# indrajeetadityaroy9/vit-bias-aware-structural-distillation

Measured on AMD Instinct MI355X. Metric: images/sec BASD train step, DeiT-T student / ViT-B teacher bs=256, higher is better.
Workload: dtype bf16; 1 GPU; BASELINE configs[1]: DeiT-Tiny/16 student, ViT-Base/16 teacher (random init), 224x224, E=4 extraction points, loss linalg fp32/fp64; global_batch=256, per_gpu_batch=256, parallelism=dp1, grad_checkpointing=False

## Files before the change

vit-bias-aware-structural-distillation_amd/csrc/attention.hip:

```cpp
#include "basd_frag.h"

namespace basd {

__device__ __forceinline__ unsigned short f32_to_bf16_rne(float f) {
  unsigned int u = __float_as_uint(f);
  u += 0x7fffu + ((u >> 16) & 1u);
  return (unsigned short)(u >> 16);
}

template <int CTRL> __device__ __forceinline__ float at_dpp_add(float v) {
  return v + __int_as_float(__builtin_amdgcn_update_dpp(0, __float_as_int(v), CTRL, 0xF, 0xF, true));
}

struct RelBias {
  const float* table;
  int gh, gw;
};


template <int NKT, int AT_HD, bool QMEAN = false, bool RELBIAS = false, bool ROPE = false>
__global__ __launch_bounds__(256) __attribute__((amdgpu_waves_per_eu(2, 2))) void attention_fwd_kernel(const unsigned short* __restrict__ qkv, int T, int H,
                                                            float scale, unsigned short* __restrict__ out,
                                                            float* __restrict__ importance, float* __restrict__ lse,
                                                            RelBias rb) {
  static_assert(!(QMEAN && RELBIAS), "the relative-position bias comes with the CLS tap only");
  static_assert(!ROPE || (!QMEAN && !RELBIAS && AT_HD == 64), "the rotary embedding: CLS tap, no bias, whole 32-deep steps");
  constexpr int NKS = (NKT + 1) / 2;
  constexpr int KROWS = 32 * NKS;
  constexpr int NDS = (AT_HD + 31) / 32;
  constexpr int NDT = AT_HD / 16;
  constexpr int NCH = AT_HD / 8;
  constexpr int NCHP = NDS * 4;
  constexpr int AT_LD = NDS * 32 + 8;
  extern __shared__ __align__(16) unsigned short sm[];
  unsigned short* Ks = sm;
  unsigned short* Vs = Ks + KROWS * AT_LD;
  unsigned short* Os = Vs + KROWS * AT_LD;
  int* koff = reinterpret_cast<int*>(Os + 4 * 16 * AT_LD);
  float* tab = reinterpret_cast<float*>(koff + KROWS);
  const int tid = threadIdx.x, lane = tid & 63, wave = tid >> 6;
  const int li = lane & 15, g = lane >> 4;
  const int b = blockIdx.x / H, h = blockIdx.x - b * H;
  const size_t row = (size_t)3 * H * AT_HD;
  const unsigned short* base = qkv + (size_t)b * T * row + (size_t)h * AT_HD;

  constexpr int NLD = (KROWS * NCHP + 255) / 256;
  uint4 kreg[NLD], vreg[NLD];
  float4 kcs[ROPE ? NLD : 1][2];
#pragma unroll
  for (int i = 0; i < NLD; ++i) {
    const int idx = tid + 256 * i;
    const int r = idx / NCHP, c8 = idx - r * NCHP;
    kreg[i] = make_uint4(0, 0, 0, 0);
    vreg[i] = make_uint4(0, 0, 0, 0);
    if constexpr (ROPE) kcs[i][0] = kcs[i][1] = make_float4(0.f, 0.f, 0.f, 0.f);
    if (r < T && c8 < NCH) {
      const unsigned short* p = base + (size_t)r * row + c8 * 8;
      kreg[i] = *reinterpret_cast<const uint4*>(p + (size_t)H * AT_HD);
      vreg[i] = *reinterpret_cast<const uint4*>(p + (size_t)2 * H * AT_HD);
      if constexpr (ROPE) {
        const float4* cs = reinterpret_cast<const float4*>(rb.table + (size_t)r * AT_HD + c8 * 8);
        kcs[i][0] = cs[0];
        kcs[i][1] = cs[1];
      }
    }
  }
  const int R = RELBIAS ? (2 * rb.gh - 1) * (2 * rb.gw - 1) + 3 : 0;
  const int rl = RELBIAS ? 2 * rb.gw - 1 : 0;
  if constexpr (RELBIAS) {
    constexpr int NTAB = (1084 + 255) / 256;
    float tv[NTAB];
#pragma unroll
    for (int i = 0; i < NTAB; ++i) tv[i] = (tid + 256 * i < R) ? rb.table[(size_t)(tid + 256 * i) * H + h] : 0.f;
#pragma unroll
    for (int i = 0; i < NTAB; ++i)
      if (tid + 256 * i < R) tab[tid + 256 * i] = tv[i];
    for (int key = tid; key < KROWS; key += 256) {
      const int yk = (key >= 1 && key < T) ? (key - 1) / rb.gw : 0;
      koff[key] = (key >= 1 && key < T) ? yk * rl + (key - 1 - yk * rb.gw) : 0;
    }
  }
#pragma unroll
  for (int i = 0; i < NLD; ++i) {
    const int idx = tid + 256 * i;
    const int r = idx / NCHP, c8 = idx - r * NCHP;
    if constexpr (ROPE) kreg[i] = rope_chunk(kreg[i], kcs[i][0], kcs[i][1]);
    if (idx < KROWS * NCHP) {
      *reinterpret_cast<uint4*>(Ks + r * AT_LD + c8 * 8) = kreg[i];
      *reinterpret_cast<uint4*>(Vs + r * AT_LD + c8 * 8) = vreg[i];
    }
  }
  __syncthreads();

  const float sl2 = RELBIAS ? 1.4426950408889634f : scale * 1.4426950408889634f;
  const int nqt = (T + 15) >> 4;
  const int full_tiles = T >> 4;
  unsigned short* Ow = Os + wave * 16 * AT_LD;
  auto load_q = [&](int qt_, uint4 (&dst)[NDS], float4 (&cs)[ROPE ? NDS : 1][2]) {
#pragma unroll
    for (int ks = 0; ks < NDS; ++ks) {
      dst[ks] = make_uint4(0, 0, 0, 0);
      if constexpr (ROPE) cs[ks][0] = cs[ks][1] = make_float4(0.f, 0.f, 0.f, 0.f);
      if (qt_ < nqt && qt_ * 16 + li < T && 32 * ks + 8 * g < AT_HD) {
        dst[ks] = *reinterpret_cast<const uint4*>(base + (size_t)(qt_ * 16 + li) * row + 32 * ks + 8 * g);
        if constexpr (ROPE) {
          const float4* p = reinterpret_cast<const float4*>(rb.table + (size_t)(qt_ * 16 + li) * AT_HD + 32 * ks + 8 * g);
          cs[ks][0] = p[0];
          cs[ks][1] = p[1];
        }
      }
    }
  };
  uint4 qnext[NDS];
  float4 qcs[ROPE ? NDS : 1][2];
  load_q(wave, qnext, qcs);
  float csum[QMEAN ? NKT : 1][4];
#pragma unroll
  for (int kt = 0; kt < (QMEAN ? NKT : 1); ++kt)
#pragma unroll
    for (int r = 0; r < 4; ++r) csum[kt][r] = 0.f;
  for (int qt = wave; qt < nqt; qt += 4) {
    const int q0 = qt * 16;
    bf16x8 qf[NDS];
#pragma unroll
    for (int ks = 0; ks < NDS; ++ks) {
      if constexpr (ROPE) qnext[ks] = rope_chunk(qnext[ks], qcs[ks][0], qcs[ks][1]);
      qf[ks] = *reinterpret_cast<bf16x8*>(&qnext[ks]);
    }
    load_q(qt + 4, qnext, qcs);
    f32x4 s[NKT];
#pragma unroll
    for (int kt = 0; kt < NKT; ++kt) {
      f32x4 acc = {0.f, 0.f, 0.f, 0.f};
#pragma unroll
      for (int ks = 0; ks < NDS; ++ks) {
        const uint4 kk = *reinterpret_cast<const uint4*>(Ks + (16 * kt + li) * AT_LD + 32 * ks + 8 * g);
        acc = __builtin_amdgcn_mfma_f32_16x16x32_bf16(*reinterpret_cast<const bf16x8*>(&kk), qf[ks], acc, 0, 0, 0);
      }
      s[kt] = acc;
      if ((kt & 3) == 3) __builtin_amdgcn_sched_barrier(0);
    }
    if constexpr (RELBIAS) {
      const int qi = q0 + li;
      const bool qcls = qi == 0 || qi >= T;
      const int yq = qcls ? 0 : (qi - 1) / rb.gw;
      const int qb = qcls ? R - 3 : (yq + rb.gh - 1) * rl + (qi - 1 - yq * rb.gw) + rb.gw - 1;
      const int c0 = qcls ? R - 1 : R - 2;
#pragma unroll
      for (int kt = 0; kt < NKT; ++kt) {
        const int4 ko = *reinterpret_cast<const int4*>(koff + 16 * kt + 4 * g);
        const int kk[4] = {ko.x, ko.y, ko.z, ko.w};
#pragma unroll
        for (int r = 0; r < 4; ++r) {
          int idx = qcls ? qb : qb - kk[r];
          if (kt == 0 && r == 0 && g == 0) idx = c0;
          s[kt][r] = fmaf(s[kt][r], scale, tab[idx]);
        }
      }
    }
    if (!QMEAN && !RELBIAS && !ROPE && importance != nullptr && qt == 0) {
      float lr[NKT][4];
      float tmx = -3.0e38f;
#pragma unroll
      for (int kt = 0; kt < NKT; ++kt)
#pragma unroll
        for (int r = 0; r < 4; r += 2) {
          const unsigned int w = pack_bf16(s[kt][r], s[kt][r + 1]);
          lr[kt][r] = __uint_as_float(w << 16) * scale;
          lr[kt][r + 1] = __uint_as_float(w & 0xffff0000u) * scale;
          if (kt >= full_tiles) {
            if (16 * kt + 4 * g + r >= T) lr[kt][r] = -3.0e38f;
            if (16 * kt + 4 * g + r + 1 >= T) lr[kt][r + 1] = -3.0e38f;
          }
          tmx = fmaxf(tmx, fmaxf(lr[kt][r], lr[kt][r + 1]));
        }
      tmx = fmaxf(tmx, __shfl_xor(tmx, 16, 64));
      tmx = fmaxf(tmx, __shfl_xor(tmx, 32, 64));
      float tsum = 0.f;
#pragma unroll
      for (int kt = 0; kt < NKT; ++kt)
#pragma unroll
        for (int r = 0; r < 4; ++r) {
          lr[kt][r] = __builtin_amdgcn_exp2f((lr[kt][r] - tmx) * 1.4426950408889634f);
          tsum += lr[kt][r];
        }
      tsum += __shfl_xor(tsum, 16, 64);
      tsum += __shfl_xor(tsum, 32, 64);
      if (li == 0) {
        const float tinv = 1.f / (tsum * (float)H);
#pragma unroll
        for (int kt = 0; kt < NKT; ++kt)
#pragma unroll
          for (int r = 0; r < 4; ++r) {
            const int key = 16 * kt + 4 * g + r;
            if (key >= 1 && (kt < full_tiles || key < T))
              importance[((size_t)b * H + h) * (T - 1) + key - 1] = lr[kt][r] * tinv;
          }
      }
    }
    float mx = -3.0e38f;
#pragma unroll
    for (int kt = 0; kt < NKT; ++kt)
#pragma unroll
      for (int r = 0; r < 4; ++r) {
        if (kt >= full_tiles && 16 * kt + 4 * g + r >= T) s[kt][r] = -3.0e38f;
        mx = fmaxf(mx, s[kt][r]);
      }
    mx = fmaxf(mx, __shfl_xor(mx, 16, 64));
    mx = fmaxf(mx, __shfl_xor(mx, 32, 64));
    float sum = 0.f;
#pragma unroll
    for (int kt = 0; kt < NKT; ++kt)
#pragma unroll
      for (int r = 0; r < 4; ++r) {
        const float p = __builtin_amdgcn_exp2f((s[kt][r] - mx) * sl2);
        s[kt][r] = p;
        sum += p;
      }
    sum += __shfl_xor(sum, 16, 64);
    sum += __shfl_xor(sum, 32, 64);
    const float inv = 1.f / sum;
    if constexpr (RELBIAS || ROPE) {
      if (importance != nullptr && qt == 0 && li == 0) {
        const float tinv = inv / (float)H;
#pragma unroll
        for (int kt = 0; kt < NKT; ++kt)
#pragma unroll
          for (int r = 0; r < 4; ++r) {
            const int key = 16 * kt + 4 * g + r;
            if (key >= 1 && key < T) importance[((size_t)b * H + h) * (T - 1) + key - 1] = s[kt][r] * tinv;
          }
      }
    }
    if constexpr (QMEAN) {
      const float qinv = (q0 + li < T) ? inv : 0.f;
#pragma unroll
      for (int kt = 0; kt < NKT; ++kt)
#pragma unroll
        for (int r = 0; r < 4; ++r) csum[kt][r] = fmaf(s[kt][r], qinv, csum[kt][r]);
    }
    if (!RELBIAS && lse != nullptr && g == 0 && q0 + li < T) lse[((size_t)b * H + h) * T + q0 + li] = fmaf(mx, scale, __logf(sum));
    f32x4 o[NDT];
#pragma unroll
    for (int dt = 0; dt < NDT; ++dt) o[dt] = (f32x4){0.f, 0.f, 0.f, 0.f};
#pragma unroll
    for (int ks = 0; ks < NKS; ++ks) {
      const int K1 = (2 * ks + 1 < NKT) ? 2 * ks + 1 : 0;
      uint4 pw;
      pw.x = pack_bf16(s[2 * ks][0] * inv, s[2 * ks][1] * inv);
      pw.y = pack_bf16(s[2 * ks][2] * inv, s[2 * ks][3] * inv);
      pw.z = (2 * ks + 1 < NKT) ? pack_bf16(s[K1][0] * inv, s[K1][1] * inv) : 0u;
      pw.w = (2 * ks + 1 < NKT) ? pack_bf16(s[K1][2] * inv, s[K1][3] * inv) : 0u;
      const bf16x8 pa = *reinterpret_cast<const bf16x8*>(&pw);
      const int qq = li >> 2, pp = li & 3;
#pragma unroll
      for (int dt = 0; dt < NDT; ++dt) {
        const unsigned short* a0 = Vs + (32 * ks + 4 * g + qq) * AT_LD + 16 * dt + 4 * pp;
        const v4s lo = __builtin_amdgcn_ds_read_tr16_b64_v4i16((lds_v4s*)a0);
        const v4s hi = __builtin_amdgcn_ds_read_tr16_b64_v4i16((lds_v4s*)(a0 + 16 * AT_LD));
        const bf16x8 vb = {lo[0], lo[1], lo[2], lo[3], hi[0], hi[1], hi[2], hi[3]};
        o[dt] = __builtin_amdgcn_mfma_f32_16x16x32_bf16(pa, vb, o[dt], 0, 0, 0);
      }
    }
#pragma unroll
    for (int dt = 0; dt < NDT; ++dt)
#pragma unroll
      for (int r = 0; r < 4; r += 2) {
        const unsigned int w = pack_bf16(o[dt][r], o[dt][r + 1]);
        Ow[(4 * g + r) * AT_LD + 16 * dt + li] = (unsigned short)(w & 0xffffu);
        Ow[(4 * g + r + 1) * AT_LD + 16 * dt + li] = (unsigned short)(w >> 16);
      }
    __builtin_amdgcn_s_waitcnt(0xc07f);
#pragma unroll
    for (int c = 0; c < (16 * NCH + 63) / 64; ++c) {
      const int idx = lane + 64 * c, r = idx / NCH, c8 = idx - r * NCH;
      if (idx < 16 * NCH && q0 + r < T) {
        const uint4 v = *reinterpret_cast<const uint4*>(Ow + r * AT_LD + c8 * 8);
        *reinterpret_cast<uint4*>(out + ((size_t)(b * T + q0 + r) * H + h) * AT_HD + c8 * 8) = v;
      }
    }
    __builtin_amdgcn_s_waitcnt(0xc07f);
  }
  if constexpr (QMEAN) {
    float* cw = reinterpret_cast<float*>(Os) + wave * (16 * AT_LD / 2);
#pragma unroll
    for (int kt = 0; kt < NKT; ++kt)
#pragma unroll
      for (int r = 0; r < 4; ++r) {
        float v = csum[kt][r];
        v = at_dpp_add<0xB1>(v);
        v = at_dpp_add<0x4E>(v);
        v = at_dpp_add<0x124>(v);
        v = at_dpp_add<0x128>(v);
        if (li == 0) cw[16 * kt + 4 * g + r] = v;
      }
    __syncthreads();
    const float* c0 = reinterpret_cast<const float*>(Os);
    const float norm = 1.f / ((float)H * (float)T);
    for (int key = tid; key < T; key += 256) {
      float v = 0.f;
#pragma unroll
      for (int w = 0; w < 4; ++w) v += c0[w * (16 * AT_LD / 2) + key];
      importance[((size_t)b * H + h) * T + key] = v * norm;
    }
  }
}

template <int NKT, int HD, bool QMEAN = false, bool RELBIAS = false, bool ROPE = false>
static void launch_attention(const void* qkv, int B, int T, int H, float scale, void* out, float* importance,
                             float* lse, hipStream_t st, RelBias rb = RelBias{nullptr, 0, 0}) {
  constexpr int KROWS = 32 * ((NKT + 1) / 2);
  constexpr int LD = (HD + 31) / 32 * 32 + 8;
  size_t lds = ((size_t)2 * KROWS * LD + 4 * 16 * LD) * sizeof(unsigned short);
  static_assert(8 * LD >= KROWS, "the output staging tile of a wave holds its query-mean column sums");
  static_assert((2 * KROWS * LD + 4 * 16 * LD) % 8 == 0, "the key offsets behind the tiles are read 16 bytes at a time");
  if (RELBIAS) lds += ((size_t)KROWS + (size_t)(2 * rb.gh - 1) * (2 * rb.gw - 1) + 3) * sizeof(float);
  allow_full_lds((const void*)attention_fwd_kernel<NKT, HD, QMEAN, RELBIAS, ROPE>);
  hipLaunchKernelGGL((attention_fwd_kernel<NKT, HD, QMEAN, RELBIAS, ROPE>), dim3(B * H), dim3(256), lds, st,
                     (const unsigned short*)qkv, T, H, scale, (unsigned short*)out, importance, lse, rb);
}

}

extern "C" int basd_attention_fwd_bf16(const void* qkv, int B, int T, int H, int hd, float scale, void* out,
                                       float* importance, float* lse, void* stream) {
  using namespace basd;
  if (B <= 0) return BASD_OK;
  if ((hd != 64 && hd != 80) || T < 1 || T > 272 || H < 1)
    return fail(BASD_ERR_SHAPE, "attention_fwd: T=%d H=%d hd=%d unsupported (hd 64 | 80, T <= 272)", T, H, hd);
  if (importance != nullptr && T < 2) return fail(BASD_ERR_SHAPE, "attention_fwd: importance needs T >= 2");
  hipStream_t st = (hipStream_t)stream;
  if (hd == 64) {
    if (T <= 64) launch_attention<4, 64>(qkv, B, T, H, scale, out, importance, lse, st);
    else if (T <= 208) launch_attention<13, 64>(qkv, B, T, H, scale, out, importance, lse, st);
    else launch_attention<17, 64>(qkv, B, T, H, scale, out, importance, lse, st);
  } else {
    if (T <= 208) launch_attention<13, 80>(qkv, B, T, H, scale, out, importance, lse, st);
    else launch_attention<17, 80>(qkv, B, T, H, scale, out, importance, lse, st);
  }
  return check_launch("attention_fwd");
}

extern "C" int basd_attention_fwd_qmean_bf16(const void* qkv, int B, int T, int H, int hd, float scale, void* out,
                                             float* importance, void* stream) {
  using namespace basd;
  if (B <= 0) return BASD_OK;
  if ((hd != 64 && hd != 80) || T < 1 || T > 272 || H < 1)
    return fail(BASD_ERR_SHAPE, "attention_fwd_qmean: T=%d H=%d hd=%d unsupported (hd 64 | 80, T <= 272)", T, H, hd);
  if (importance == nullptr) return fail(BASD_ERR_SHAPE, "attention_fwd_qmean: importance is required");
  hipStream_t st = (hipStream_t)stream;
  if (hd == 64) {
    if (T <= 64) launch_attention<4, 64, true>(qkv, B, T, H, scale, out, importance, nullptr, st);
    else if (T <= 208) launch_attention<13, 64, true>(qkv, B, T, H, scale, out, importance, nullptr, st);
    else launch_attention<17, 64, true>(qkv, B, T, H, scale, out, importance, nullptr, st);
  } else {
    if (T <= 208) launch_attention<13, 80, true>(qkv, B, T, H, scale, out, importance, nullptr, st);
    else launch_attention<17, 80, true>(qkv, B, T, H, scale, out, importance, nullptr, st);
  }
  return check_launch("attention_fwd_qmean");
}

extern "C" int basd_attention_fwd_relbias_bf16(const void* qkv, const float* table, int B, int gh, int gw, int H, int hd,
                                               float scale, void* out, float* importance, void* stream) {
  using namespace basd;
  if (hd != 64 || gh < 1 || gw < 1 || gh > 271 || gw > 271 || gh * gw > 271 || H < 1)
    return fail(BASD_ERR_SHAPE, "attention_fwd_relbias: grid %d x %d H=%d hd=%d unsupported (hd 64, 2 <= gh * gw + 1 <= 272)",
                gh, gw, H, hd);
  if (B <= 0) return BASD_OK;
  const int T = gh * gw + 1;
  const RelBias rb{table, gh, gw};
  hipStream_t st = (hipStream_t)stream;
  if (T <= 64) launch_attention<4, 64, false, true>(qkv, B, T, H, scale, out, importance, nullptr, st, rb);
  else if (T <= 208) launch_attention<13, 64, false, true>(qkv, B, T, H, scale, out, importance, nullptr, st, rb);
  else launch_attention<17, 64, false, true>(qkv, B, T, H, scale, out, importance, nullptr, st, rb);
  return check_launch("attention_fwd_relbias");
}

extern "C" int basd_attention_fwd_rope_bf16(const void* qkv, const float* rope, int B, int T, int H, int hd, float scale,
                                            void* out, float* importance, void* stream) {
  using namespace basd;
  if (hd != 64 || T < 2 || T > 272 || H < 1 || B < 1 || rope == nullptr)
    return fail(BASD_ERR_SHAPE, "attention_fwd_rope: B=%d T=%d H=%d hd=%d rope=%s unsupported (hd 64, 2 <= T <= 272, B, H >= 1, "
                                "a table)", B, T, H, hd, rope == nullptr ? "NULL" : "given");
  const RelBias rb{rope, 0, 0};
  hipStream_t st = (hipStream_t)stream;
  if (T <= 64) launch_attention<4, 64, false, false, true>(qkv, B, T, H, scale, out, importance, nullptr, st, rb);
  else if (T <= 208) launch_attention<13, 64, false, false, true>(qkv, B, T, H, scale, out, importance, nullptr, st, rb);
  else launch_attention<17, 64, false, false, true>(qkv, B, T, H, scale, out, importance, nullptr, st, rb);
  return check_launch("attention_fwd_rope");
}
```

Measured before the change: 8161 images/sec.

## Software-pipeline K/V LDS reads, rebalance query tiles, and coalesce importance stores

Result: no change. 8181 images/sec (median of 6 runs) (+0.2%).

```diff
diff --git a/vit-bias-aware-structural-distillation_amd/csrc/attention.hip b/vit-bias-aware-structural-distillation_amd/csrc/attention.hip
--- a/vit-bias-aware-structural-distillation_amd/csrc/attention.hip
+++ b/vit-bias-aware-structural-distillation_amd/csrc/attention.hip
@@ -32,6 +32,10 @@
   constexpr int NCH = AT_HD / 8;
   constexpr int NCHP = NDS * 4;
   constexpr int AT_LD = NDS * 32 + 8;
+  constexpr bool TIGHT = NKT == 17 && AT_HD == 80;
+  constexpr int KD = TIGHT ? (QMEAN ? 1 : 2) : 4;
+  constexpr int VD = TIGHT ? (QMEAN ? 0 : 1) : 2;
+  constexpr int SCHED_PIN = 0x2 | 0x4 | 0x10 | 0x400;
   extern __shared__ __align__(16) unsigned short sm[];
   unsigned short* Ks = sm;
   unsigned short* Vs = Ks + KROWS * AT_LD;
@@ -65,37 +69,10 @@
       }
     }
   }
-  const int R = RELBIAS ? (2 * rb.gh - 1) * (2 * rb.gw - 1) + 3 : 0;
-  const int rl = RELBIAS ? 2 * rb.gw - 1 : 0;
-  if constexpr (RELBIAS) {
-    constexpr int NTAB = (1084 + 255) / 256;
-    float tv[NTAB];
-#pragma unroll
-    for (int i = 0; i < NTAB; ++i) tv[i] = (tid + 256 * i < R) ? rb.table[(size_t)(tid + 256 * i) * H + h] : 0.f;
-#pragma unroll
-    for (int i = 0; i < NTAB; ++i)
-      if (tid + 256 * i < R) tab[tid + 256 * i] = tv[i];
-    for (int key = tid; key < KROWS; key += 256) {
-      const int yk = (key >= 1 && key < T) ? (key - 1) / rb.gw : 0;
-      koff[key] = (key >= 1 && key < T) ? yk * rl + (key - 1 - yk * rb.gw) : 0;
-    }
-  }
-#pragma unroll
-  for (int i = 0; i < NLD; ++i) {
-    const int idx = tid + 256 * i;
-    const int r = idx / NCHP, c8 = idx - r * NCHP;
-    if constexpr (ROPE) kreg[i] = rope_chunk(kreg[i], kcs[i][0], kcs[i][1]);
-    if (idx < KROWS * NCHP) {
-      *reinterpret_cast<uint4*>(Ks + r * AT_LD + c8 * 8) = kreg[i];
-      *reinterpret_cast<uint4*>(Vs + r * AT_LD + c8 * 8) = vreg[i];
-    }
-  }
-  __syncthreads();
-
-  const float sl2 = RELBIAS ? 1.4426950408889634f : scale * 1.4426950408889634f;
   const int nqt = (T + 15) >> 4;
-  const int full_tiles = T >> 4;
-  unsigned short* Ow = Os + wave * 16 * AT_LD;
+  const int nround = nqt >> 2;
+  const int wextra = 4 * nround + ((wave + 3) & 3);
+  auto tile_of = [&](int i) { return (QMEAN || i < nround) ? wave + 4 * i : (i == nround ? wextra : nqt); };
   auto load_q = [&](int qt_, uint4 (&dst)[NDS], float4 (&cs)[ROPE ? NDS : 1][2]) {
 #pragma unroll
     for (int ks = 0; ks < NDS; ++ks) {
@@ -113,13 +90,58 @@
   };
   uint4 qnext[NDS];
   float4 qcs[ROPE ? NDS : 1][2];
-  load_q(wave, qnext, qcs);
+  load_q(tile_of(0), qnext, qcs);
+  const int R = RELBIAS ? (2 * rb.gh - 1) * (2 * rb.gw - 1) + 3 : 0;
+  const int rl = RELBIAS ? 2 * rb.gw - 1 : 0;
+  if constexpr (RELBIAS) {
+    constexpr int NTAB = (1084 + 255) / 256;
+    float tv[NTAB];
+#pragma unroll
+    for (int i = 0; i < NTAB; ++i) tv[i] = (tid + 256 * i < R) ? rb.table[(size_t)(tid + 256 * i) * H + h] : 0.f;
+#pragma unroll
+    for (int i = 0; i < NTAB; ++i)
+      if (tid + 256 * i < R) tab[tid + 256 * i] = tv[i];
+    for (int key = tid; key < KROWS; key += 256) {
+      const int yk = (key >= 1 && key < T) ? (key - 1) / rb.gw : 0;
+      koff[key] = (key >= 1 && key < T) ? yk * rl + (key - 1 - yk * rb.gw) : 0;
+    }
+  }
+#pragma unroll
+  for (int i = 0; i < NLD; ++i) {
+    const int idx = tid + 256 * i;
+    const int r = idx / NCHP, c8 = idx - r * NCHP;
+    if constexpr (ROPE) kreg[i] = rope_chunk(kreg[i], kcs[i][0], kcs[i][1]);
+    if (idx < KROWS * NCHP) {
+      *reinterpret_cast<uint4*>(Ks + r * AT_LD + c8 * 8) = kreg[i];
+      *reinterpret_cast<uint4*>(Vs + r * AT_LD + c8 * 8) = vreg[i];
+    }
+  }
+  __syncthreads();
+
+  const float sl2 = RELBIAS ? 1.4426950408889634f : scale * 1.4426950408889634f;
+  const int full_tiles = T >> 4;
+  unsigned short* Ow = Os + wave * 16 * AT_LD;
+  auto store_tap = [&](const float (&v)[NKT][4]) {
+    float* tw = reinterpret_cast<float*>(Ow);
+    if (li == 0) {
+#pragma unroll
+      for (int kt = 0; kt < NKT; ++kt)
+        *reinterpret_cast<float4*>(tw + 16 * kt + 4 * g) = make_float4(v[kt][0], v[kt][1], v[kt][2], v[kt][3]);
+    }
+    __builtin_amdgcn_s_waitcnt(0xc07f);
+#pragma unroll
+    for (int c = 0; c < (16 * NKT + 63) / 64; ++c) {
+      const int key = lane + 64 * c;
+      if (key >= 1 && key < T) importance[((size_t)b * H + h) * (T - 1) + key - 1] = tw[key];
+    }
+    __builtin_amdgcn_s_waitcnt(0xc07f);
+  };
   float csum[QMEAN ? NKT : 1][4];
 #pragma unroll
   for (int kt = 0; kt < (QMEAN ? NKT : 1); ++kt)
 #pragma unroll
     for (int r = 0; r < 4; ++r) csum[kt][r] = 0.f;
-  for (int qt = wave; qt < nqt; qt += 4) {
+  for (int it = 0, qt = tile_of(0); qt < nqt; qt = tile_of(++it)) {
     const int q0 = qt * 16;
     bf16x8 qf[NDS];
 #pragma unroll
@@ -127,19 +149,41 @@
       if constexpr (ROPE) qnext[ks] = rope_chunk(qnext[ks], qcs[ks][0], qcs[ks][1]);
       qf[ks] = *reinterpret_cast<bf16x8*>(&qnext[ks]);
     }
-    load_q(qt + 4, qnext, qcs);
+    load_q(tile_of(it + 1), qnext, qcs);
     f32x4 s[NKT];
+    uint4 kf[NKT][NDS];
+    auto read_k = [&](int kt) {
+#pragma unroll
+      for (int ks = 0; ks < NDS; ++ks)
+        kf[kt][ks] = *reinterpret_cast<const uint4*>(Ks + (16 * kt + li) * AT_LD + 32 * ks + 8 * g);
+    };
+#pragma unroll
+    for (int kt = 0; kt < KD && kt < NKT; ++kt) read_k(kt);
 #pragma unroll
     for (int kt = 0; kt < NKT; ++kt) {
+      if (kt + KD < NKT) read_k(kt + KD);
+      __builtin_amdgcn_sched_barrier(SCHED_PIN);
       f32x4 acc = {0.f, 0.f, 0.f, 0.f};
 #pragma unroll
-      for (int ks = 0; ks < NDS; ++ks) {
-        const uint4 kk = *reinterpret_cast<const uint4*>(Ks + (16 * kt + li) * AT_LD + 32 * ks + 8 * g);
-        acc = __builtin_amdgcn_mfma_f32_16x16x32_bf16(*reinterpret_cast<const bf16x8*>(&kk), qf[ks], acc, 0, 0, 0);
-      }
+      for (int ks = 0; ks < NDS; ++ks)
+        acc = __builtin_amdgcn_mfma_f32_16x16x32_bf16(*reinterpret_cast<const bf16x8*>(&kf[kt][ks]), qf[ks], acc, 0, 0, 0);
       s[kt] = acc;
-      if ((kt & 3) == 3) __builtin_amdgcn_sched_barrier(0);
-    }
+      __builtin_amdgcn_sched_barrier(SCHED_PIN);
+    }
+    bf16x8 vf[NKS][NDT];
+    const int qq = li >> 2, pp = li & 3;
+    auto read_v = [&](int ks) {
+#pragma unroll
+      for (int dt = 0; dt < NDT; ++dt) {
+        const unsigned short* a0 = Vs + (32 * ks + 4 * g + qq) * AT_LD + 16 * dt + 4 * pp;
+        const v4s lo = __builtin_amdgcn_ds_read_tr16_b64_v4i16((lds_v4s*)a0);
+        const v4s hi = __builtin_amdgcn_ds_read_tr16_b64_v4i16((lds_v4s*)(a0 + 16 * AT_LD));
+        vf[ks][dt] = (bf16x8){lo[0], lo[1], lo[2], lo[3], hi[0], hi[1], hi[2], hi[3]};
+      }
+    };
+#pragma unroll
+    for (int ks = 0; ks < VD && ks < NKS; ++ks) read_v(ks);
+    __builtin_amdgcn_sched_barrier(SCHED_PIN);
     if constexpr (RELBIAS) {
       const int qi = q0 + li;
       const bool qcls = qi == 0 || qi >= T;
@@ -186,17 +230,12 @@
         }
       tsum += __shfl_xor(tsum, 16, 64);
       tsum += __shfl_xor(tsum, 32, 64);
-      if (li == 0) {
-        const float tinv = 1.f / (tsum * (float)H);
-#pragma unroll
-        for (int kt = 0; kt < NKT; ++kt)
-#pragma unroll
-          for (int r = 0; r < 4; ++r) {
-            const int key = 16 * kt + 4 * g + r;
-            if (key >= 1 && (kt < full_tiles || key < T))
-              importance[((size_t)b * H + h) * (T - 1) + key - 1] = lr[kt][r] * tinv;
-          }
-      }
+      const float tinv = 1.f / (tsum * (float)H);
+#pragma unroll
+      for (int kt = 0; kt < NKT; ++kt)
+#pragma unroll
+        for (int r = 0; r < 4; ++r) lr[kt][r] *= tinv;
+      store_tap(lr);
     }
     float mx = -3.0e38f;
 #pragma unroll
@@ -221,15 +260,14 @@
     sum += __shfl_xor(sum, 32, 64);
     const float inv = 1.f / sum;
     if constexpr (RELBIAS || ROPE) {
-      if (importance != nullptr && qt == 0 && li == 0) {
+      if (importance != nullptr && qt == 0) {
         const float tinv = inv / (float)H;
+        float tp[NKT][4];
 #pragma unroll
         for (int kt = 0; kt < NKT; ++kt)
 #pragma unroll
-          for (int r = 0; r < 4; ++r) {
-            const int key = 16 * kt + 4 * g + r;
-            if (key >= 1 && key < T) importance[((size_t)b * H + h) * (T - 1) + key - 1] = s[kt][r] * tinv;
-          }
+          for (int r = 0; r < 4; ++r) tp[kt][r] = s[kt][r] * tinv;
+        store_tap(tp);
       }
     }
     if constexpr (QMEAN) {
@@ -252,15 +290,11 @@
       pw.z = (2 * ks + 1 < NKT) ? pack_bf16(s[K1][0] * inv, s[K1][1] * inv) : 0u;
       pw.w = (2 * ks + 1 < NKT) ? pack_bf16(s[K1][2] * inv, s[K1][3] * inv) : 0u;
       const bf16x8 pa = *reinterpret_cast<const bf16x8*>(&pw);
-      const int qq = li >> 2, pp = li & 3;
-#pragma unroll
-      for (int dt = 0; dt < NDT; ++dt) {
-        const unsigned short* a0 = Vs + (32 * ks + 4 * g + qq) * AT_LD + 16 * dt + 4 * pp;
-        const v4s lo = __builtin_amdgcn_ds_read_tr16_b64_v4i16((lds_v4s*)a0);
-        const v4s hi = __builtin_amdgcn_ds_read_tr16_b64_v4i16((lds_v4s*)(a0 + 16 * AT_LD));
-        const bf16x8 vb = {lo[0], lo[1], lo[2], lo[3], hi[0], hi[1], hi[2], hi[3]};
-        o[dt] = __builtin_amdgcn_mfma_f32_16x16x32_bf16(pa, vb, o[dt], 0, 0, 0);
-      }
+      if (ks + VD < NKS) read_v(ks + VD);
+      __builtin_amdgcn_sched_barrier(SCHED_PIN);
+#pragma unroll
+      for (int dt = 0; dt < NDT; ++dt) o[dt] = __builtin_amdgcn_mfma_f32_16x16x32_bf16(pa, vf[ks][dt], o[dt], 0, 0, 0);
+      __builtin_amdgcn_sched_barrier(SCHED_PIN);
     }
 #pragma unroll
     for (int dt = 0; dt < NDT; ++dt)
```
